# AllanYangZhou/midGPT

Hardware: AMD Instinct MI355X
Metric: tokens_per_sec (higher is better)
Workload: dtype bf16; 1 GPU; model=openwebtext_xl-gpt-1311M, global_batch=128, seq_len=1024, parallelism=dp1, g_accum_iters=2, remat=False

## Files before the change

midgpt_amd/ops/csrc/attention.hip:

```cpp
#include "common.h"
#include "mfma.h"
#include "philox.h"

struct AttnStrides {
  long b, h;
  int r;
};
DEVINL long bh_base(const AttnStrides& s, long bh, int H) {
  return (bh / H) * s.b + (bh % H) * s.h;
}

template <int C> DEVINL int swz_rm(int row, int byte_in_row) {
  constexpr int M = (C == 128) ? 15 : 7;
  return byte_in_row ^ ((row & M) << 4);
}
DEVINL int swz_tr(int row, int byte_in_row) {
  return byte_in_row ^ (((row >> 2) & 3) << 4);
}

template <int C, int NT>
struct RmStage {
  static constexpr int NV = (32 * C + NT * 8 - 1) / (NT * 8);
  u16x8 v[NV];
  DEVINL void load(const u16* __restrict__ g, int ld = C) {
    static_assert((NT * 8) % C == 0, "a thread keeps its column across loads");
    const int idx0 = threadIdx.x * 8;
    const unsigned boff = 2u * (unsigned)((idx0 / C) * ld + idx0 % C);
#pragma unroll
    for (int i = 0; i < NV; ++i) {
      if (idx0 + i * NT * 8 < 32 * C)
        v[i] = *(const u16x8*)((const char*)(g + (long)(i * (NT * 8 / C)) * ld) + boff);
    }
  }
  DEVINL void write(u16* lds) const {
#pragma unroll
    for (int i = 0; i < NV; ++i) {
      const int idx = threadIdx.x * 8 + i * NT * 8;
      if (idx < 32 * C) {
        const int row = idx / C, col = idx % C;
        *(u16x8*)((char*)lds + row * C * 2 + swz_rm<C>(row, col * 2)) = v[i];
      }
    }
  }
};
template <int C, int NT, bool ACCK = false>
struct TrStage {
  static constexpr int NP = (32 * C + NT * 16 - 1) / (NT * 16);
  u16x8 a[NP], b[NP];
  DEVINL void load(const u16* __restrict__ g, int ld = C) {
    static_assert((NT * 8) % C == 0, "a thread keeps its column across loads");
    const int idx0 = threadIdx.x * 16;
    const unsigned boff =
        2u * (unsigned)(2 * (idx0 / (2 * C)) * ld + (idx0 / 2) % C);
#pragma unroll
    for (int i = 0; i < NP; ++i) {
      if (idx0 + i * NT * 16 >= 32 * C) continue;
      const u16* gi = g + (long)(i * 2 * (NT * 8 / C)) * ld;
      const char* pa = (const char*)gi + boff;
      int ldb = 2 * ld;
      asm volatile("" : "+s"(ldb));
      if constexpr (ACCK) {
        unsigned off = boff;
        asm volatile("" : "+v"(off));
        a[i] = *(const u16x8*)((const char*)gi + off);
        b[i] = *(const u16x8*)((const char*)gi + ldb + off);
        continue;
      }
      a[i] = *(const u16x8*)pa;
      b[i] = *(const u16x8*)(pa + ldb);
    }
  }
  DEVINL void write_tr(u16* lds) const {
#pragma unroll
    for (int i = 0; i < NP; ++i) {
      const int idx = threadIdx.x * 16 + i * NT * 16;
      if (idx >= 32 * C) continue;
      const int row0 = 2 * (idx / (2 * C));
      const int row = ACCK ? acc_k_pos(row0) : row0;
      const int col = (idx / 2) % C;
      if constexpr (ACCK) {
        const u32x4 aw = __builtin_bit_cast(u32x4, a[i]);
        const u32x4 bw = __builtin_bit_cast(u32x4, b[i]);
        const int x = (row * 2) ^ (((col >> 3) & 1) << 5);
        char* const p0 = (char*)lds + col * 64 + x;
        char* const p1 = (char*)lds + col * 64 + (x ^ 16);
#pragma unroll
        for (int j = 0; j < 8; ++j) {
          const unsigned pv = (j & 1)
              ? (aw[j >> 1] >> 16) | (bw[j >> 1] & 0xffff0000u)
              : (aw[j >> 1] & 0xffffu) | (bw[j >> 1] << 16);
          *(unsigned*)((j < 4 ? p0 : p1) + j * 64) = pv;
        }
        continue;
      }
#pragma unroll
      for (int j = 0; j < 8; ++j) {
        const int r = col + j;
        u16x2 pv; pv.x = a[i][j]; pv.y = b[i][j];
        *(u16x2*)((char*)lds + r * 64 + swz_tr(r, row * 2)) = pv;
      }
    }
  }
  DEVINL void write_rm(u16* lds) const {
#pragma unroll
    for (int i = 0; i < NP; ++i) {
      const int idx = threadIdx.x * 16 + i * NT * 16;
      if (idx >= 32 * C) continue;
      const int row = 2 * (idx / (2 * C));
      const int col = (idx / 2) % C;
      *(u16x8*)((char*)lds + row * C * 2 + swz_rm<C>(row, col * 2)) = a[i];
      *(u16x8*)((char*)lds + (row + 1) * C * 2 + swz_rm<C>(row + 1, col * 2)) = b[i];
    }
  }
};
template <int C, int NT>
DEVINL void stage_rm(const u16* __restrict__ g, u16* lds, int ld = C) {
  RmStage<C, NT> st; st.load(g, ld); st.write(lds);
}
template <int C, int NT, bool ACCK = false>
DEVINL void stage_tr(const u16* __restrict__ g, u16* lds, int ld = C) {
  TrStage<C, NT, ACCK> st; st.load(g, ld); st.write_tr(lds);
}

template <int C>
DEVINL bf16x8_t read_rm_frag(const u16* lds, int row, int cbyte) {
  return *(const bf16x8_t*)((const char*)lds + row * C * 2 + swz_rm<C>(row, cbyte));
}
DEVINL bf16x8_t read_tr_frag(const u16* lds, int row, int kbyte) {
  return *(const bf16x8_t*)((const char*)lds + row * 64 + swz_tr(row, kbyte));
}

DEVINL float shfl32(float v, int src) { return __shfl(v, src, 32); }

template <int C, int NW, int SPW, bool DROP = false>
__global__ __launch_bounds__(NW * 64, 2) void attn_fwd_kernel(const u16* __restrict__ q,
                                const u16* __restrict__ k,
                                const u16* __restrict__ v,
                                u16* __restrict__ o, float* __restrict__ lse,
                                int B, int H, int T,
                                AttnStrides sv, AttnStrides so,
                                uint32_t seed_lo = 0, uint32_t seed_hi = 0,
                                uint32_t drop_thr = 0, float inv_keep = 1.f) {
  constexpr int NCB = C / 32;
  constexpr int NCH = C / 16;
  constexpr int NSTRIP = NW * SPW;
  const float scale = rsqrtf((float)C);
  const long bh = blockIdx.x % ((long)B * H);
  const int qb = blockIdx.x / (B * H);
  const int q0 = qb * (NSTRIP * 32);
  const int lane = lane_id();
  const int w = wave_id();
  int strip[SPW];
  strip[0] = w;
  if (SPW == 2) strip[1] = NSTRIP - 1 - w;

  extern __shared__ __attribute__((aligned(16))) char smem[];
  u16* ldsK = (u16*)smem;
  u16* ldsVt = (u16*)(smem + 2 * 32 * C * 2);
  float* obuf = (float*)smem;

  const u16* qg = q + (bh * T) * C;
  const u16* kg = k + (bh * T) * C;
  const u16* vg = v + bh_base(sv, bh, H);

  bf16x8_t qf[NCH];
  f32x16 oacc[SPW][NCB];
  float m[SPW], lsum[SPW];
  {
    const u16* qrow = qg + (long)(q0 + 32 * strip[SPW - 1] + (lane & 31)) * C;
#pragma unroll
    for (int ch = 0; ch < NCH; ++ch)
      qf[ch] = *(const bf16x8_t*)(qrow + 16 * ch + 8 * (lane >> 5));
  }
#pragma unroll
  for (int sp = 0; sp < SPW; ++sp) {
#pragma unroll
    for (int cb = 0; cb < NCB; ++cb) oacc[sp][cb] = (f32x16)(0.f);
    m[sp] = -1e30f;
    lsum[sp] = 0.f;
  }

  const int nkt = (q0 + NSTRIP * 32) / 32;
  stage_rm<C, NW * 64>(kg, ldsK);
  stage_tr<C, NW * 64>(vg, ldsVt, sv.r);
  __syncthreads();

  RmStage<C, NW * 64> kst;
  TrStage<C, NW * 64> vst;
  for (int kt = 0; kt < nkt; ++kt) {
    const int buf = kt & 1;
    const bool pre = kt + 1 < nkt;
    if (pre) {
      kst.load(kg + (long)(kt + 1) * 32 * C);
      vst.load(vg + (long)(kt + 1) * 32 * sv.r, sv.r);
    }
    const int k0 = kt * 32;
#pragma unroll
    for (int sp = 0; sp < SPW; ++sp) {
      const int qw0 = q0 + 32 * strip[sp];
      const int myq = qw0 + (lane & 31);
      if (k0 > qw0 + 31) continue;
      f32x16 s = (f32x16)(0.f);
      const u16* kb = ldsK + buf * 32 * C;
      const u16* qrow = qg + (long)myq * C;
#pragma unroll
      for (int ch = 0; ch < NCH; ++ch) {
        bf16x8_t a = read_rm_frag<C>(kb, lane & 31, 16 * ch * 2 + 16 * (lane >> 5));
        bf16x8_t qfr = (sp == SPW - 1) ? qf[ch]
            : *(const bf16x8_t*)(qrow + 16 * ch + 8 * (lane >> 5));
        s = mfma_32x32x16_bf16(a, qfr, s);
      }
      float sv[16];
      float mt = -1e30f;
#pragma unroll
      for (int r = 0; r < 16; ++r) {
        sv[r] = (k0 + mfma_d_row(lane, r) > myq) ? -1e30f : s[r];
        mt = fmaxf(mt, sv[r]);
      }
      mt = fmaxf(mt, __shfl_xor(mt, 32));
      const float mn = fmaxf(m[sp], mt);
      const float alpha = __expf((m[sp] - mn) * scale);
      const bool need_rescale = !__all(mt <= m[sp]);
      m[sp] = mn;
      float p[16], psum = 0.f;
#pragma unroll
      for (int r = 0; r < 16; ++r) {
        p[r] = __expf((sv[r] - mn) * scale);
        psum += p[r];
      }
      psum += __shfl_xor(psum, 32);
      lsum[sp] = lsum[sp] * alpha + psum;
      if (need_rescale) {
        float arow[16];
#pragma unroll
        for (int r = 0; r < 16; ++r) arow[r] = shfl32(alpha, mfma_d_row(lane, r));
#pragma unroll
        for (int cb = 0; cb < NCB; ++cb)
#pragma unroll
// ... 32 lines not shown
      vst.write_tr(ldsVt + (1 - buf) * C * 32);
    }
    __syncthreads();
  }

#pragma unroll
  for (int sp = 0; sp < SPW; ++sp) {
    const int qw0 = q0 + 32 * strip[sp];
    const int myq = qw0 + (lane & 31);
    float rec = 1.f / lsum[sp];
    if constexpr (DROP) rec *= inv_keep;
    float rrow[16];
#pragma unroll
    for (int r = 0; r < 16; ++r) rrow[r] = shfl32(rec, mfma_d_row(lane, r));
    if (lane < 32) lse[bh * T + myq] = m[sp] * scale + __logf(lsum[sp]);
    float* ob = obuf + w * 32 * 32;
    u16* og = o + bh_base(so, bh, H) + (long)qw0 * so.r;
#pragma unroll
    for (int cb = 0; cb < NCB; ++cb) {
#pragma unroll
      for (int r = 0; r < 16; ++r) {
        const int row = mfma_d_row(lane, r);
        *(float*)((char*)ob + row * 128 + (((lane & 31) * 4) ^ ((row & 7) << 4))) =
            oacc[sp][cb][r] * rrow[r];
      }
      __builtin_amdgcn_s_waitcnt(0);
      const int row = lane & 31;
      const int c16 = 16 * (lane >> 5);
      float tmp[16];
#pragma unroll
      for (int i = 0; i < 4; ++i) {
        f32x4 t = *(const f32x4*)((char*)ob + row * 128 + (((c16 + 4 * i) * 4) ^ ((row & 7) << 4)));
        tmp[4 * i] = t[0]; tmp[4 * i + 1] = t[1]; tmp[4 * i + 2] = t[2]; tmp[4 * i + 3] = t[3];
      }
      u16x8 out0, out1;
#pragma unroll
      for (int j = 0; j < 8; ++j) { out0[j] = f2b(tmp[j]); out1[j] = f2b(tmp[8 + j]); }
      *(u16x8*)(og + (long)row * so.r + 32 * cb + c16) = out0;
      *(u16x8*)(og + (long)row * so.r + 32 * cb + c16 + 8) = out1;
      __builtin_amdgcn_s_waitcnt(0);
    }
  }
}

template <int C, int NW>
__global__ __launch_bounds__(NW * 64, 2) void attn_fwd2_kernel(
    const u16* __restrict__ q, const u16* __restrict__ k,
    const u16* __restrict__ v, u16* __restrict__ o, float* __restrict__ lse,
    int B, int H, int T, AttnStrides sv, AttnStrides so) {
  constexpr int NCB = C / 32;
  constexpr int NCH = C / 16;
  const float scale = rsqrtf((float)C);
  const long bh = blockIdx.x % ((long)B * H);
  const int qb = blockIdx.x / (B * H);
  const int q0 = qb * (NW * 32);
  const int lane = lane_id();
  const int w = wave_id();
  const int qw0 = q0 + 32 * w;
  const int myq = qw0 + (lane & 31);

  extern __shared__ __attribute__((aligned(16))) char smem[];
  u16* ldsK = (u16*)smem;
  u16* ldsVt = (u16*)(smem + 2 * 64 * C * 2);
  float* obuf = (float*)smem;

  const u16* qg = q + (bh * T) * C;
  const u16* kg = k + (bh * T) * C;
  const u16* vg = v + bh_base(sv, bh, H);

  bf16x8_t qf[NCH];
  {
    const u16* qrow = qg + (long)myq * C;
#pragma unroll
    for (int ch = 0; ch < NCH; ++ch)
      qf[ch] = *(const bf16x8_t*)(qrow + 16 * ch + 8 * (lane >> 5));
  }
  f32x16 oacc[NCB];
#pragma unroll
  for (int cb = 0; cb < NCB; ++cb) oacc[cb] = (f32x16)(0.f);
  float m = -1e30f, lsum = 0.f;

  const int nrounds = (q0 + NW * 32) / 64;
  stage_rm<C, NW * 64>(kg, ldsK);
  stage_rm<C, NW * 64>(kg + 32 * C, ldsK + 32 * C);
  stage_tr<C, NW * 64>(vg, ldsVt, sv.r);
  stage_tr<C, NW * 64>(vg + (long)32 * sv.r, ldsVt + C * 32, sv.r);
  __syncthreads();

  RmStage<C, NW * 64> kstA, kstB;
  TrStage<C, NW * 64> vstA, vstB;
  for (int rd = 0; rd < nrounds; ++rd) {
    const int buf = rd & 1;
    const bool pre = rd + 1 < nrounds;
    if (pre) {
      const long nb = (long)(rd + 1) * 64;
      kstA.load(kg + nb * C);
      kstB.load(kg + (nb + 32) * C);
      vstA.load(vg + nb * sv.r, sv.r);
      vstB.load(vg + (nb + 32) * sv.r, sv.r);
    }
    const int k0 = rd * 64;
    if (k0 <= qw0 + 31) {
      const u16* kbuf = ldsK + buf * 64 * C;
      const u16* vbuf = ldsVt + buf * 64 * C;
      const bool needB = (k0 + 32) <= qw0 + 31;
      f32x16 s0 = (f32x16)(0.f), s1 = (f32x16)(0.f);
#pragma unroll
      for (int ch = 0; ch < NCH; ++ch) {
        bf16x8_t a0 = read_rm_frag<C>(kbuf, lane & 31, 16 * ch * 2 + 16 * (lane >> 5));
        s0 = mfma_32x32x16_bf16(a0, qf[ch], s0);
      }
      if (needB) {
#pragma unroll
        for (int ch = 0; ch < NCH; ++ch) {
          bf16x8_t a1 = read_rm_frag<C>(kbuf + 32 * C, lane & 31,
                                        16 * ch * 2 + 16 * (lane >> 5));
          s1 = mfma_32x32x16_bf16(a1, qf[ch], s1);
        }
      }
      float sv0[16], sv1[16];
      float mt = -1e30f;
#pragma unroll
      for (int r = 0; r < 16; ++r) {
        sv0[r] = (k0 + mfma_d_row(lane, r) > myq) ? -1e30f : s0[r];
        mt = fmaxf(mt, sv0[r]);
        sv1[r] = (!needB || k0 + 32 + mfma_d_row(lane, r) > myq) ? -1e30f : s1[r];
        mt = fmaxf(mt, sv1[r]);
      }
      mt = fmaxf(mt, __shfl_xor(mt, 32));
      const float mn = fmaxf(m, mt);
      const float alpha = __expf((m - mn) * scale);
      const bool need_rescale = !__all(mt <= m);
      m = mn;
      float p0[16], p1[16], psum = 0.f;
#pragma unroll
      for (int r = 0; r < 16; ++r) {
        p0[r] = __expf((sv0[r] - mn) * scale);
        p1[r] = __expf((sv1[r] - mn) * scale);
        psum += p0[r] + p1[r];
      }
// ... 99 lines not shown
      bh = urow / (unsigned)T;
      t = urow % (unsigned)T;
    }
    const u16* dor = dO + bh_base(sdo, bh, H) + t * sdo.r;
    const u16* orow = O + bh_base(so, bh, H) + t * so.r;
    float acc = 0.f;
    const u16x8 a = *(const u16x8*)(dor + i);
    const u16x8 b = *(const u16x8*)(orow + i);
    if (do_copy) *(u16x8*)(do_copy + (bh * T + t) * C + i) = a;
#pragma unroll
    for (int j = 0; j < 8; ++j) acc += b2f(a[j]) * b2f(b[j]);
    acc = group_sum<LPR>(acc);
    if (lane % LPR == 0) delta[bh * T + t] = acc;
  }
}

template <int C, int NW>
constexpr bool attn_dkv_vf_lds = !(C == 128 && NW == 4);
template <int C, int NW>
constexpr int attn_dkv_kf_lds = C == 128 ? 3 : 0;

template <int C, int NW, bool DROP = false>
__global__ __launch_bounds__(NW * 64, 2) void attn_bwd_dkv_kernel(
    const u16* __restrict__ dO, const u16* __restrict__ q,
    const u16* __restrict__ k, const u16* __restrict__ v,
    const float* __restrict__ lse, const float* __restrict__ delta,
    u16* __restrict__ dk, u16* __restrict__ dv, int B, int H, int T,
    AttnStrides sdo, AttnStrides sv, AttnStrides sdv,
    uint32_t seed_lo = 0, uint32_t seed_hi = 0, uint32_t drop_thr = 0,
    float inv_keep = 1.f) {
  constexpr int NCB = C / 32;
  constexpr int NCH = C / 16;
  constexpr int TILE = 4 * 32 * C;
  const float scale = rsqrtf((float)C);
  const long bh = blockIdx.x % ((long)B * H);
  const int kb = blockIdx.x / (B * H);
  const int lane = lane_id();
  const int w = wave_id();
  const int kw0 = kb * (NW * 32) + 32 * w;
  const int myk = kw0 + (lane & 31);

  extern __shared__ __attribute__((aligned(16))) char smem[];
  u16* base = (u16*)smem;
  float* ldsLse = (float*)(base + 2 * TILE);
  float* ldsDelta = ldsLse + 64;
  constexpr bool VF_LDS = attn_dkv_vf_lds<C, NW>;
  bf16x8_t* ldsVf = (bf16x8_t*)(ldsDelta + 64) + w * (NCH * 64) + lane;

  const u16* qg = q + (bh * T) * C;
  const u16* kg = k + (bh * T) * C;
  const u16* vg = v + bh_base(sv, bh, H);
  const u16* dog = dO + bh_base(sdo, bh, H);
  const u16* krow = kg + (long)myk * C;
  const u16* vrow = vg + (long)myk * sv.r;
  if constexpr (VF_LDS) {
#pragma unroll
    for (int ch = 0; ch < NCH; ++ch)
      ldsVf[ch * 64] = *(const bf16x8_t*)(vrow + 16 * ch + 8 * (lane >> 5));
  }

  constexpr bool KF_RES = !(DROP && C == 128);
  constexpr int NKL = KF_RES ? attn_dkv_kf_lds<C, NW> : 0;
  constexpr int NKR = KF_RES ? NCH - NKL : 0;
  bf16x8_t kf[NKR ? NKR : 1];
  bf16x8_t* ldsKf = (bf16x8_t*)(ldsDelta + 64) + (VF_LDS ? NW * (NCH * 64) : 0) +
                    w * (NKL * 64) + lane;
  if (KF_RES) {
#pragma unroll
    for (int ch = 0; ch < NCH; ++ch) {
      const bf16x8_t f = *(const bf16x8_t*)(krow + 16 * ch + 8 * (lane >> 5));
      if (ch < NKR) kf[ch < NKR ? ch : 0] = f;
      else ldsKf[(ch - NKR) * 64] = f;
    }
  }

  f32x16 dvacc[NCB], dkacc[NCB];
#pragma unroll
  for (int cb = 0; cb < NCB; ++cb) { dvacc[cb] = (f32x16)(0.f); dkacc[cb] = (f32x16)(0.f); }

  const int qt0 = kb * NW;
  const int nqt = T / 32;

  auto stage_set = [&](int qt, int buf) {
    const long qbase = (long)qt * 32;
    u16* bq = base + buf * TILE;
    stage_rm<C, NW * 64>(qg + qbase * C, bq);
    stage_tr<C, NW * 64, true>(qg + qbase * C, bq + 32 * C);
    stage_rm<C, NW * 64>(dog + qbase * sdo.r, bq + 2 * 32 * C, sdo.r);
    stage_tr<C, NW * 64, true>(dog + qbase * sdo.r, bq + 3 * 32 * C, sdo.r);
    if (threadIdx.x < 32) {
      ldsLse[buf * 32 + threadIdx.x] = lse[bh * T + qbase + threadIdx.x];
      ldsDelta[buf * 32 + threadIdx.x] = delta[bh * T + qbase + threadIdx.x];
    }
  };

  stage_set(qt0, 0);
  __syncthreads();
  __builtin_amdgcn_s_waitcnt(0);
  TrStage<C, NW * 64, true> qst, dost;
  float lse_r = 0.f, del_r = 0.f;
  for (int qt = qt0; qt < nqt; ++qt) {
    const int buf = (qt - qt0) & 1;
    const bool pre = qt + 1 < nqt;
    if (pre) {
      const long nb = (long)(qt + 1) * 32;
      qst.load(qg + nb * C);
      dost.load(dog + nb * sdo.r, sdo.r);
      if (threadIdx.x < 32) {
        unsigned off = 4u * threadIdx.x;
        asm volatile("" : "+v"(off));
        lse_r = *(const float*)((const char*)(lse + bh * T + nb) + off);
        del_r = *(const float*)((const char*)(delta + bh * T + nb) + off);
      }
    }
    const int qbase = qt * 32;
    if (qbase + 31 >= kw0) {
      const u16* ldsQ = base + buf * TILE;
      const u16* ldsQt = ldsQ + 32 * C;
      const u16* ldsDO = ldsQt + C * 32;
      const u16* ldsDOt = ldsDO + 32 * C;
      const float* lseb = ldsLse + buf * 32;
      const float* deltab = ldsDelta + buf * 32;
      uint32_t keep = 0;
      if constexpr (DROP) {
#pragma unroll
        for (int g = 0; g < 4; ++g)
          keep |= attn_drop_keep4(seed_lo, seed_hi, (uint32_t)bh,
                                  (uint32_t)(qbase + 8 * g + 4 * (lane >> 5)) >> 2,
                                  (uint32_t)myk, drop_thr) << (4 * g);
        __builtin_amdgcn_sched_barrier(0);
      }
      f32x16 s = (f32x16)(0.f);
#pragma unroll
      for (int ch = 0; ch < NCH; ++ch) {
        bf16x8_t a = read_rm_frag<C>(ldsQ, lane & 31, 16 * ch * 2 + 16 * (lane >> 5));
        bf16x8_t kfr;
        if constexpr (!KF_RES) kfr = *(const bf16x8_t*)(krow + 16 * ch + 8 * (lane >> 5));
        else if (ch < NKR) kfr = kf[ch < NKR ? ch : 0];
        else kfr = ldsKf[(ch - NKR) * 64];
        s = mfma_32x32x16_bf16(a, kfr, s);
      }
      float p[16];
#pragma unroll
      for (int g = 0; g < 4; ++g) {
        const f32x4 l4 = *(const f32x4*)(lseb + 8 * g + 4 * (lane >> 5));
#pragma unroll
        for (int i = 0; i < 4; ++i) {
          const int r = 4 * g + i;
          const int qrow = qbase + mfma_d_row(lane, r);
          p[r] = (myk > qrow) ? 0.f : __expf(s[r] * scale - l4[i]);
        }
      }
      const bf16x8_t pf0 = dlayout_pack(p, DROP ? keep : 0xffu);
      const bf16x8_t pf1 = dlayout_pack(p + 8, DROP ? keep >> 8 : 0xffu);
#pragma unroll
      for (int cb = 0; cb < NCB; ++cb) {
        bf16x8_t b0 = read_tr_frag(ldsDOt, 32 * cb + (lane & 31), 16 * (lane >> 5));
        bf16x8_t b1 = read_tr_frag(ldsDOt, 32 * cb + (lane & 31), 32 + 16 * (lane >> 5));
        dvacc[cb] = mfma_32x32x16_bf16(pf0, b0, dvacc[cb]);
        dvacc[cb] = mfma_32x32x16_bf16(pf1, b1, dvacc[cb]);
      }
      f32x16 dp = (f32x16)(0.f);
#pragma unroll
      for (int ch = 0; ch < NCH; ++ch) {
        bf16x8_t a = read_rm_frag<C>(ldsDO, lane & 31, 16 * ch * 2 + 16 * (lane >> 5));
        bf16x8_t vf;
        if constexpr (VF_LDS) vf = ldsVf[ch * 64];
        else vf = *(const bf16x8_t*)(vrow + 16 * ch + 8 * (lane >> 5));
        dp = mfma_32x32x16_bf16(a, vf, dp);
      }
      float ds[16];
#pragma unroll
      for (int g = 0; g < 4; ++g) {
        const f32x4 d4 = *(const f32x4*)(deltab + 8 * g + 4 * (lane >> 5));
#pragma unroll
        for (int i = 0; i < 4; ++i) {
          const int r = 4 * g + i;
          float dpr = dp[r];
          if constexpr (DROP) dpr = ((keep >> r) & 1u) ? dpr * inv_keep : 0.f;
          ds[r] = p[r] * (dpr - d4[i]) * scale;
        }
      }
      const bf16x8_t df0 = dlayout_pack(ds);
      const bf16x8_t df1 = dlayout_pack(ds + 8);
#pragma unroll
      for (int cb = 0; cb < NCB; ++cb) {
        bf16x8_t b0 = read_tr_frag(ldsQt, 32 * cb + (lane & 31), 16 * (lane >> 5));
        bf16x8_t b1 = read_tr_frag(ldsQt, 32 * cb + (lane & 31), 32 + 16 * (lane >> 5));
        dkacc[cb] = mfma_32x32x16_bf16(df0, b0, dkacc[cb]);
        dkacc[cb] = mfma_32x32x16_bf16(df1, b1, dkacc[cb]);
      }
    }
    if (pre) {
      u16* bq = base + (buf ^ 1) * TILE;
      qst.write_rm(bq);
      qst.write_tr(bq + 32 * C);
      dost.write_rm(bq + 2 * 32 * C);
      dost.write_tr(bq + 3 * 32 * C);
      if (threadIdx.x < 32) {
        ldsLse[(buf ^ 1) * 32 + threadIdx.x] = lse_r;
        ldsDelta[(buf ^ 1) * 32 + threadIdx.x] = del_r;
      }
    }
    __syncthreads();
  }

  float* ob = (float*)smem + w * 32 * 32;
  u16* dkg = dk + (bh * T + kw0) * C;
  u16* dvg = dv + bh_base(sdv, bh, H) + (long)kw0 * sdv.r;
#pragma unroll
  for (int which = 0; which < 2; ++which) {
    f32x16* acc = which == 0 ? dkacc : dvacc;
    u16* out = which == 0 ? dkg : dvg;
    const int old = which == 0 ? C : sdv.r;
#pragma unroll
    for (int cb = 0; cb < NCB; ++cb) {
#pragma unroll
      for (int r = 0; r < 16; ++r) {
        const int row = mfma_d_row(lane, r);
        float a = acc[cb][r];
        if constexpr (DROP) { if (which == 1) a *= inv_keep; }
        *(float*)((char*)ob + row * 128 + (((lane & 31) * 4) ^ ((row & 7) << 4))) = a;
      }
      __builtin_amdgcn_s_waitcnt(0);
      const int row = lane & 31;
      const int c16 = 16 * (lane >> 5);
      float tmp[16];
#pragma unroll
      for (int i = 0; i < 4; ++i) {
        f32x4 t = *(const f32x4*)((char*)ob + row * 128 +
                                  (((c16 + 4 * i) * 4) ^ ((row & 7) << 4)));
        tmp[4 * i] = t[0]; tmp[4 * i + 1] = t[1];
        tmp[4 * i + 2] = t[2]; tmp[4 * i + 3] = t[3];
      }
      u16x8 o0, o1;
#pragma unroll
      for (int j = 0; j < 8; ++j) { o0[j] = f2b(tmp[j]); o1[j] = f2b(tmp[8 + j]); }
// ... 181 lines not shown
```

midgpt_amd/ops/csrc/bindings.cpp:

```cpp
#include <torch/extension.h>
#include <hip/hip_runtime.h>
#include <c10/hip/HIPGuard.h>
#include <c10/hip/HIPStream.h>

#include <algorithm>
#include <climits>
#include <type_traits>
#include <vector>

static hipStream_t cur_stream() { return c10::hip::getCurrentHIPStream().stream(); }

template <typename... P, typename... A>
static void launch(void (*kernel)(P...), dim3 grid, int block, size_t smem, A... args) {
  if (grid.x == 0 || grid.y == 0 || grid.z == 0) return;
  if (smem > 64 * 1024) {
    hipError_t e = hipFuncSetAttribute(reinterpret_cast<const void*>(kernel),
                                       hipFuncAttributeMaxDynamicSharedMemorySize, (int)smem);
    TORCH_CHECK(e == hipSuccess, "cannot raise dynamic LDS to ", smem, " bytes: ",
                hipGetErrorString(e));
  }
  hipLaunchKernelGGL(kernel, grid, dim3(block), smem, cur_stream(), static_cast<P>(args)...);
  hipError_t e = hipGetLastError();
  TORCH_CHECK(e == hipSuccess, "HIP launch failed: ", hipGetErrorString(e));
}
// ... 23 lines not shown
      if (sizes[i] != ANY && sizes[i] != ts[i]) return false;
    return true;
  }
};
static Shape flat(int64_t n) {
  Shape s((at::IntArrayRef()));
  s.numel = n;
  return s;
}
static std::ostream& operator<<(std::ostream& o, const Shape& s) {
  return s.numel >= 0 ? o << s.numel << " elements" : o << "shape " << s.sizes << " (-1: any)";
}

template <typename T>
static T* fresh(const torch::Tensor& t) {
  return static_cast<T*>(t.data_ptr());
}

struct Call {
  const char* who;
  int dev;
  c10::hip::OptionalHIPGuard guard;

  static int device_of(const char* who, const torch::Tensor& first) {
    TORCH_CHECK(first.defined() && first.is_cuda(), who, ": the first tensor must be on the GPU");
    return first.get_device();
  }
  Call(const char* who, const torch::Tensor& first) : who(who), dev(device_of(who, first)) {
    if (dev != c10::hip::current_device()) guard.set_index((c10::DeviceIndex)dev);
  }

  template <typename T, c10::ScalarType ST>
  T* ptr(const torch::Tensor& t, const char* name, const Shape& s) const {
    TORCH_CHECK(t.defined() && t.is_cuda() && t.get_device() == dev,
                who, ": ", name, " must be a tensor on GPU ", dev);
    TORCH_CHECK(t.is_contiguous() && t.scalar_type() == ST && s.fits(t),
                who, ": ", name, " must be contiguous ", ST, " of ", s, ", got ",
                t.scalar_type(), " ", t.sizes(), t.is_contiguous() ? "" : " (strided)");
    return static_cast<T*>(t.data_ptr());
  }
  const u16* bf16(const torch::Tensor& t, const char* n, const Shape& s) const {
    return ptr<u16, torch::kBFloat16>(t, n, s);
  }
  u16* bf16_out(const torch::Tensor& t, const char* n, const Shape& s) const {
    return ptr<u16, torch::kBFloat16>(t, n, s);
  }
  const float* f32(const torch::Tensor& t, const char* n, const Shape& s) const {
    return ptr<float, torch::kFloat>(t, n, s);
  }
  float* f32_out(const torch::Tensor& t, const char* n, const Shape& s) const {
    return ptr<float, torch::kFloat>(t, n, s);
  }
  const long* i64(const torch::Tensor& t, const char* n, const Shape& s) const {
    return ptr<long, torch::kLong>(t, n, s);
  }
  const int* i32(const torch::Tensor& t, const char* n, const Shape& s) const {
    return ptr<int, torch::kInt>(t, n, s);
  }
  const u16* bf16(const c10::optional<torch::Tensor>& t, const char* n, const Shape& s) const {
    return t.has_value() ? bf16(*t, n, s) : nullptr;
  }
  int dim(const torch::Tensor& t, int i) const {
    const int64_t n = t.sizes()[i];
    TORCH_CHECK(n <= INT_MAX, who, ": a dimension of ", n, " does not fit int");
    return (int)n;
  }
};

std::vector<torch::Tensor> rmsnorm_fwd(torch::Tensor x, c10::optional<torch::Tensor> w,
                                       double eps) {
  Call c("rmsnorm_fwd", x);
  const bool fp32 = x.scalar_type() == torch::kFloat;
  const float* xf = fp32 ? c.f32(x, "x", {ANY, ANY}) : nullptr;
  const u16* xb = fp32 ? nullptr : c.bf16(x, "x", {ANY, ANY});
  long N = x.size(0);
  int D = c.dim(x, 1);
  TORCH_CHECK(fp32 || D % 8 == 0, "rmsnorm_fwd: bf16 rows need D % 8 == 0");
  auto y = torch::empty_like(x);
  auto invrms = torch::empty({N}, x.options().dtype(torch::kFloat));
  const float* wp = nullptr;
  torch::Tensor wf;
  if (w.has_value()) {
    wf = w->to(torch::kFloat).contiguous();
    wp = c.f32(wf, "w", flat(D));
  }
  int rows_per_block = 4;
  long grid = std::min((N + rows_per_block - 1) / rows_per_block, (long)8192);
  if (fp32)
    launch(rmsnorm_fwd_kernel<float, 1>, grid, 256, 0, xf, wp, fresh<float>(y),
           fresh<float>(invrms), N, D, (float)eps);
  else
    launch(rmsnorm_fwd_bf16, grid, 256, 0, xb, wp, fresh<u16>(y), fresh<float>(invrms), N, D,
           (float)eps);
  return {y, invrms};
}

std::vector<torch::Tensor> rmsnorm_bwd(torch::Tensor dy, torch::Tensor x,
                                       c10::optional<torch::Tensor> w,
                                       torch::Tensor invrms, double eps) {
  Call c("rmsnorm_bwd", dy);
  TORCH_CHECK(!w.has_value(), "rmsnorm_bwd: weighted path unimplemented on HIP "
                              "(the model's norms are weightless)");
  const u16* xp = c.bf16(x, "x", {ANY, ANY});
  long N = x.size(0);
  int D = c.dim(x, 1);
  TORCH_CHECK(D % 8 == 0, "rmsnorm_bwd: D % 8 == 0 required");
// ... 891 lines not shown
  auto out = torch::empty({(long)B}, logits.options().dtype(torch::kLong));
  const bool has_k = top_k >= 1 && top_k < V;
  const uint64_t s = (uint64_t)seed;
  dispatch_flag(has_k, [&](auto hk) {
    launch(sample_tokens_kernel<decltype(hk)::value>, B, SAMPLE_THREADS, 0, lp,
           fresh<long>(out), V, it, has_k ? (int)top_k : 0, (uint32_t)s, (uint32_t)(s >> 32),
           (uint32_t)step);
  });
  return out;
}

torch::Tensor sample_tokens_rows(torch::Tensor logits, torch::Tensor params_dev,
                                 torch::Tensor inv_t, torch::Tensor top_k, torch::Tensor seeds,
                                 torch::Tensor steps, torch::Tensor rows) {
  Call c("sample_tokens_rows", logits);
  const u16* lp = c.bf16(logits, "logits", {ANY, ANY});
  const int B = c.dim(logits, 0), V = c.dim(logits, 1);
  TORCH_CHECK(V >= 1, "sample_tokens_rows: empty rows");
  TORCH_CHECK(!inv_t.is_cuda() && inv_t.dim() == 1 && inv_t.size(0) == B &&
              inv_t.scalar_type() == torch::kFloat,
              c.who, ": inv_t must be a CPU float32 tensor of ", B, " values");
  auto itc = inv_t.contiguous();
  for (int b = 0; b < B; ++b) {
    const float it = itc.data_ptr<float>()[b];
    TORCH_CHECK(std::isfinite(it) && it >= 0.f, c.who,
                ": inv_t must be finite and > 0, or 0 for a greedy row, got ", it);
  }
  for (int64_t k : host_lens(top_k, B, c.who))
    TORCH_CHECK(k >= 0, c.who, ": top_k >= 0 required (0: all), got ", k);
  host_lens(seeds, B, c.who);
  for (int64_t s : host_lens(steps, B, c.who))
    TORCH_CHECK(s >= 0 && s <= (int64_t)UINT32_MAX, c.who, ": step must be in [0, 2^32), got ", s);
  for (int64_t r : host_lens(rows, B, c.who))
    TORCH_CHECK(r >= 0 && r <= (int64_t)UINT32_MAX, c.who, ": row must be in [0, 2^32), got ", r);
  const int* pp = c.i32(params_dev, "params_dev", {B, SAMPLE_ROW_WORDS});
  auto out = torch::empty({(long)B}, logits.options().dtype(torch::kLong));
  launch(sample_tokens_rows_kernel, B, SAMPLE_THREADS, 0, lp, fresh<long>(out), V, pp);
  return out;
}

torch::Tensor probe_mfma(torch::Tensor A, torch::Tensor B) {
  Call c("probe_mfma", A);
  const float *ap = c.f32(A, "A", {32, 16}), *bp = c.f32(B, "B", {16, 32});
  auto D = torch::zeros({32, 32}, A.options());
  launch(probe_mfma_kernel, 1, 64, 0, ap, bp, fresh<float>(D));
  return D;
}
torch::Tensor probe_pack(torch::Tensor M, torch::Tensor B) {
  Call c("probe_pack", M);
  const float *mp = c.f32(M, "M", {32, 32}), *bp = c.f32(B, "B", {32, 32});
  auto D = torch::zeros({32, 32}, M.options());
  launch(probe_pack_kernel, 1, 64, 0, mp, bp, fresh<float>(D));
  return D;
}

#include "blaslt.inc"

PYBIND11_MODULE(TORCH_EXTENSION_NAME, mod) {
  mod.def("rmsnorm_fwd", &rmsnorm_fwd);
  mod.def("rmsnorm_bwd", &rmsnorm_bwd);
  mod.def("qkv_prep_fwd", &qkv_prep_fwd);
  mod.def("qkv_prep_bwd", &qkv_prep_bwd);
  mod.def("add_rmsnorm_fwd", &add_rmsnorm_fwd);
  mod.def("add_rmsnorm_bwd", &add_rmsnorm_bwd);
  mod.def("qk_prep_fwd", &qk_prep_fwd);
  mod.def("qk_prep_bwd", &qk_prep_bwd);
  mod.def("ce_fwd", &ce_fwd);
  mod.def("ce_bwd", &ce_bwd);
  mod.def("adamw_step", &adamw_step);
  mod.def("attn_fwd", &attn_fwd);
  mod.def("attn_bwd", &attn_bwd);
  mod.def("attn_delta", &attn_delta, py::arg("dO"), py::arg("o"), py::arg("bthc"));
  mod.def("attn_fwd_dropout", &attn_fwd_dropout);
  mod.def("attn_bwd_dropout", &attn_bwd_dropout);
  mod.def("attn_fwd_packed", &attn_fwd_packed, py::arg("q"), py::arg("k"),
          py::arg("v"), py::arg("p") = 0.0, py::arg("seed") = 0);
  mod.def("attn_bwd_packed", &attn_bwd_packed, py::arg("dO"), py::arg("q"),
          py::arg("k"), py::arg("v"), py::arg("o"), py::arg("lse"),
          py::arg("dqkv"), py::arg("p") = 0.0, py::arg("seed") = 0,
          py::arg("stage_do") = true);
  mod.def("kv_append", &kv_append, py::arg("qkv"), py::arg("qw"), py::arg("kw"),
          py::arg("sin"), py::arg("cos"), py::arg("k_cache"), py::arg("v_cache"),
          py::arg("pos"), py::arg("eps") = 1e-6);
  mod.def("attn_decode", &attn_decode, py::arg("q"), py::arg("k_cache"),
          py::arg("v_cache"), py::arg("kv_len"), py::arg("num_splits") = 0);
  mod.def("kv_append_ragged", &kv_append_ragged, py::arg("qkv"), py::arg("qw"),
          py::arg("kw"), py::arg("sin"), py::arg("cos"), py::arg("k_cache"),
          py::arg("v_cache"), py::arg("pos_dev"), py::arg("pos_host"),
          py::arg("eps") = 1e-6);
  mod.def("attn_decode_ragged", &attn_decode_ragged, py::arg("q"), py::arg("k_cache"),
          py::arg("v_cache"), py::arg("kv_lens_dev"), py::arg("kv_lens_host"),
          py::arg("num_splits") = 0);
  mod.def("kv_append_slots", &kv_append_slots, py::arg("qkv"), py::arg("qw"), py::arg("kw"),
          py::arg("sin"), py::arg("cos"), py::arg("k_cache"), py::arg("v_cache"),
          py::arg("pos_dev"), py::arg("pos_host"), py::arg("slots_dev"),
          py::arg("slots_host"), py::arg("eps") = 1e-6);
  mod.def("attn_decode_slots", &attn_decode_slots, py::arg("q"), py::arg("k_cache"),
          py::arg("v_cache"), py::arg("kv_lens_dev"), py::arg("kv_lens_host"),
          py::arg("slots_dev"), py::arg("slots_host"), py::arg("num_splits") = 0);
  mod.def("kv_append_paged", &kv_append_paged, py::arg("qkv"), py::arg("qw"), py::arg("kw"),
          py::arg("sin"), py::arg("cos"), py::arg("k_pool"), py::arg("v_pool"),
          py::arg("pos_dev"), py::arg("pos_host"), py::arg("block_table_dev"),
          py::arg("block_table_host"), py::arg("eps") = 1e-6);
  mod.def("attn_decode_paged", &attn_decode_paged, py::arg("q"), py::arg("k_pool"),
          py::arg("v_pool"), py::arg("kv_lens_dev"), py::arg("kv_lens_host"),
          py::arg("block_table_dev"), py::arg("block_table_host"), py::arg("num_splits") = 0);
  mod.def("kv_store_paged", &kv_store_paged, py::arg("k"), py::arg("v"), py::arg("k_pool"),
          py::arg("v_pool"), py::arg("lens_dev"), py::arg("lens_host"),
          py::arg("block_table_dev"), py::arg("block_table_host"));
  mod.def("attn_decode_auto_splits", &attn_decode_auto_splits, py::arg("rows"),
          py::arg("kv_len"), py::arg("cus"));
  mod.def("sample_tokens", &sample_tokens, py::arg("logits"), py::arg("inv_t"),
          py::arg("top_k"), py::arg("seed"), py::arg("step"));
  mod.def("sample_tokens_rows", &sample_tokens_rows, py::arg("logits"), py::arg("params_dev"),
          py::arg("inv_t"), py::arg("top_k"), py::arg("seeds"), py::arg("steps"),
          py::arg("rows"));
  mod.def("embedding_bwd", &embedding_bwd);
  mod.def("gelu_fwd", &gelu_fwd);
  mod.def("gelu_bwd", &gelu_bwd);
  mod.def("transpose_batched", &transpose_batched, py::arg("src"), py::arg("dst"),
          py::arg("table_dev"), py::arg("table_host"), py::arg("max_blocks") = 0);
  mod.def("lt_probe", &lt_probe);
  mod.def("matmul_dgelu", &matmul_dgelu);
  mod.def("probe_mfma", &probe_mfma);
  mod.def("probe_pack", &probe_pack);
}
```

midgpt_amd/ops/csrc/mfma.h:

```cpp
#pragma once
#include "common.h"

using bf16x8_t = __attribute__((ext_vector_type(8))) __bf16;

DEVINL f32x16 mfma_32x32x16_bf16(bf16x8_t a, bf16x8_t b, f32x16 c) {
  return __builtin_amdgcn_mfma_f32_32x32x16_bf16(a, b, c, 0, 0, 0);
}

DEVINL int mfma_d_row(int lane, int r) {
  return (r & 3) + 8 * (r >> 2) + 4 * (lane >> 5);
}

DEVINL unsigned pack_bf16(float lo, float hi) {
  return ((unsigned)f2b(hi) << 16) | (unsigned)f2b(lo);
}

DEVINL int acc_k_pos(int i) {
  return (i & ~12) | ((i & 4) << 1) | ((i & 8) >> 1);
}

DEVINL bf16x8_t dlayout_pack(const float* s , unsigned keep8 = 0xffu) {
  union { unsigned u[4]; bf16x8_t v; } out;
#pragma unroll
  for (int i = 0; i < 4; ++i) {
    const unsigned mk = (((keep8 >> (2 * i)) & 1u) ? 0x0000ffffu : 0u) |
                        (((keep8 >> (2 * i + 1)) & 1u) ? 0xffff0000u : 0u);
    out.u[i] = pack_bf16(s[2 * i], s[2 * i + 1]) & mk;
  }
  return out.v;
}

DEVINL bf16x8_t dlayout_to_afrag(const float* s ) {
  unsigned x0 = pack_bf16(s[0], s[1]);
  unsigned x1 = pack_bf16(s[2], s[3]);
  unsigned x2 = pack_bf16(s[4], s[5]);
  unsigned x3 = pack_bf16(s[6], s[7]);
  {
    auto r = __builtin_amdgcn_permlane32_swap(x0, x2, false, false);
    x0 = r[0]; x2 = r[1];
  }
  {
    auto r = __builtin_amdgcn_permlane32_swap(x1, x3, false, false);
    x1 = r[0]; x3 = r[1];
  }
  union { unsigned u[4]; bf16x8_t v; } out;
  out.u[0] = x0; out.u[1] = x1; out.u[2] = x2; out.u[3] = x3;
  return out.v;
}
```

midgpt_amd/ops/csrc/probe.hip:

```cpp
#include "common.h"
#include "mfma.h"

__global__ void probe_mfma_kernel(const float* __restrict__ A,
                                  const float* __restrict__ B,
                                  float* __restrict__ D) {
  const int lane = threadIdx.x;
  bf16x8_t a, b;
#pragma unroll
  for (int j = 0; j < 8; ++j) {
    a[j] = (__bf16)A[(lane & 31) * 16 + 8 * (lane >> 5) + j];
    b[j] = (__bf16)B[(8 * (lane >> 5) + j) * 32 + (lane & 31)];
  }
  f32x16 d = (f32x16)(0.f);
  d = mfma_32x32x16_bf16(a, b, d);
#pragma unroll
  for (int r = 0; r < 16; ++r)
    D[mfma_d_row(lane, r) * 32 + (lane & 31)] = d[r];
}

__global__ void probe_pack_kernel(const float* __restrict__ M,
                                  const float* __restrict__ B,
                                  float* __restrict__ D) {
  const int lane = threadIdx.x;
  float m[16];
#pragma unroll
  for (int r = 0; r < 16; ++r)
    m[r] = M[mfma_d_row(lane, r) * 32 + (lane & 31)];
  bf16x8_t a0 = dlayout_to_afrag(m);
  bf16x8_t a1 = dlayout_to_afrag(m + 8);
  bf16x8_t b0, b1;
#pragma unroll
  for (int j = 0; j < 8; ++j) {
    b0[j] = (__bf16)B[(8 * (lane >> 5) + j) * 32 + (lane & 31)];
    b1[j] = (__bf16)B[(16 + 8 * (lane >> 5) + j) * 32 + (lane & 31)];
  }
  f32x16 d = (f32x16)(0.f);
  d = mfma_32x32x16_bf16(a0, b0, d);
  d = mfma_32x32x16_bf16(a1, b1, d);
#pragma unroll
  for (int r = 0; r < 16; ++r)
    D[mfma_d_row(lane, r) * 32 + (lane & 31)] = d[r];
}
```

Measured before the change: 121,000 tokens/s.

## Tune attention kernels: reverse causal block order, packed bf16 convert, scheduling barriers

Several unrelated attention tweaks land together. The staging loops are split into unconditional full iterations plus one guarded tail, and the transpose write always uses the word-packed path. The second forward kernel launches the heaviest causal query blocks first, and pack_bf16 uses a vector convert that may lower to a packed bf16 conversion instruction. The backward pass adds sched_barriers and asm pins around the P and dS packs and keeps V loads as offsets. Extra waitcnts after the initial barriers and a bf16 pack probe kernel are also added. The changed non-ACCK transpose write path may not match the old swz_tr layout.

Result: faster. 124,800 tokens/s, median of 6 (+3.2%).

```diff
diff --git a/midgpt_amd/ops/csrc/attention.hip b/midgpt_amd/ops/csrc/attention.hip
--- a/midgpt_amd/ops/csrc/attention.hip
+++ b/midgpt_amd/ops/csrc/attention.hip
@@ -21,95 +21,103 @@
 template <int C, int NT>
 struct RmStage {
   static constexpr int NV = (32 * C + NT * 8 - 1) / (NT * 8);
+  static constexpr int NF = (32 * C) / (NT * 8);
   u16x8 v[NV];
+  DEVINL void load1(const u16* __restrict__ g, int ld, unsigned boff, int i) {
+    v[i] = *(const u16x8*)((const char*)(g + (long)(i * (NT * 8 / C)) * ld) + boff);
+  }
   DEVINL void load(const u16* __restrict__ g, int ld = C) {
     static_assert((NT * 8) % C == 0, "a thread keeps its column across loads");
     const int idx0 = threadIdx.x * 8;
     const unsigned boff = 2u * (unsigned)((idx0 / C) * ld + idx0 % C);
 #pragma unroll
-    for (int i = 0; i < NV; ++i) {
-      if (idx0 + i * NT * 8 < 32 * C)
-        v[i] = *(const u16x8*)((const char*)(g + (long)(i * (NT * 8 / C)) * ld) + boff);
-    }
+    for (int i = 0; i < NF; ++i) load1(g, ld, boff, i);
+    if constexpr (NV > NF) {
+      if (idx0 + NF * NT * 8 < 32 * C) load1(g, ld, boff, NF);
+    }
+  }
+  DEVINL void write1(u16* lds, int i) const {
+    const int idx = threadIdx.x * 8 + i * NT * 8;
+    const int row = idx / C, col = idx % C;
+    *(u16x8*)((char*)lds + row * C * 2 + swz_rm<C>(row, col * 2)) = v[i];
   }
   DEVINL void write(u16* lds) const {
 #pragma unroll
-    for (int i = 0; i < NV; ++i) {
-      const int idx = threadIdx.x * 8 + i * NT * 8;
-      if (idx < 32 * C) {
-        const int row = idx / C, col = idx % C;
-        *(u16x8*)((char*)lds + row * C * 2 + swz_rm<C>(row, col * 2)) = v[i];
-      }
+    for (int i = 0; i < NF; ++i) write1(lds, i);
+    if constexpr (NV > NF) {
+      if ((int)threadIdx.x * 8 + NF * NT * 8 < 32 * C) write1(lds, NF);
     }
   }
 };
 template <int C, int NT, bool ACCK = false>
 struct TrStage {
   static constexpr int NP = (32 * C + NT * 16 - 1) / (NT * 16);
+  static constexpr int NF = (32 * C) / (NT * 16);
+  static DEVINL bool mine(int i) { return (int)threadIdx.x * 16 + i * NT * 16 < 32 * C; }
   u16x8 a[NP], b[NP];
+  DEVINL void load1(const u16* __restrict__ g, int ld, unsigned boff, int i) {
+    const u16* gi = g + (long)(i * 2 * (NT * 8 / C)) * ld;
+    int ldb = 2 * ld;
+    asm volatile("" : "+s"(ldb));
+    if constexpr (ACCK) {
+      unsigned off = boff;
+      asm volatile("" : "+v"(off));
+      a[i] = *(const u16x8*)((const char*)gi + off);
+      b[i] = *(const u16x8*)((const char*)gi + ldb + off);
+    } else {
+      const char* pa = (const char*)gi + boff;
+      a[i] = *(const u16x8*)pa;
+      b[i] = *(const u16x8*)(pa + ldb);
+    }
+  }
   DEVINL void load(const u16* __restrict__ g, int ld = C) {
     static_assert((NT * 8) % C == 0, "a thread keeps its column across loads");
     const int idx0 = threadIdx.x * 16;
     const unsigned boff =
         2u * (unsigned)(2 * (idx0 / (2 * C)) * ld + (idx0 / 2) % C);
 #pragma unroll
-    for (int i = 0; i < NP; ++i) {
-      if (idx0 + i * NT * 16 >= 32 * C) continue;
-      const u16* gi = g + (long)(i * 2 * (NT * 8 / C)) * ld;
-      const char* pa = (const char*)gi + boff;
-      int ldb = 2 * ld;
-      asm volatile("" : "+s"(ldb));
-      if constexpr (ACCK) {
-        unsigned off = boff;
-        asm volatile("" : "+v"(off));
-        a[i] = *(const u16x8*)((const char*)gi + off);
-        b[i] = *(const u16x8*)((const char*)gi + ldb + off);
-        continue;
-      }
-      a[i] = *(const u16x8*)pa;
-      b[i] = *(const u16x8*)(pa + ldb);
+    for (int i = 0; i < NF; ++i) load1(g, ld, boff, i);
+    if constexpr (NP > NF) {
+      if (mine(NF)) load1(g, ld, boff, NF);
+    }
+  }
+  DEVINL void write_tr1(u16* lds, int i) const {
+    const int idx = threadIdx.x * 16 + i * NT * 16;
+    const int row0 = 2 * (idx / (2 * C));
+    const int row = ACCK ? acc_k_pos(row0) : row0;
+    const int col = (idx / 2) % C;
+    const u32x4 aw = __builtin_bit_cast(u32x4, a[i]);
+    const u32x4 bw = __builtin_bit_cast(u32x4, b[i]);
+    const int x = (row * 2) ^ (((col >> 3) & 1) << 5);
+    char* const p0 = (char*)lds + col * 64 + x;
+    char* const p1 = (char*)lds + col * 64 + (x ^ 16);
+#pragma unroll
+    for (int j = 0; j < 8; ++j) {
+      const unsigned pv = (j & 1)
+          ? (aw[j >> 1] >> 16) | (bw[j >> 1] & 0xffff0000u)
+          : (aw[j >> 1] & 0xffffu) | (bw[j >> 1] << 16);
+      *(unsigned*)((j < 4 ? p0 : p1) + j * 64) = pv;
     }
   }
   DEVINL void write_tr(u16* lds) const {
 #pragma unroll
-    for (int i = 0; i < NP; ++i) {
-      const int idx = threadIdx.x * 16 + i * NT * 16;
-      if (idx >= 32 * C) continue;
-      const int row0 = 2 * (idx / (2 * C));
-      const int row = ACCK ? acc_k_pos(row0) : row0;
-      const int col = (idx / 2) % C;
-      if constexpr (ACCK) {
-        const u32x4 aw = __builtin_bit_cast(u32x4, a[i]);
-        const u32x4 bw = __builtin_bit_cast(u32x4, b[i]);
-        const int x = (row * 2) ^ (((col >> 3) & 1) << 5);
-        char* const p0 = (char*)lds + col * 64 + x;
-        char* const p1 = (char*)lds + col * 64 + (x ^ 16);
-#pragma unroll
-        for (int j = 0; j < 8; ++j) {
-          const unsigned pv = (j & 1)
-              ? (aw[j >> 1] >> 16) | (bw[j >> 1] & 0xffff0000u)
-              : (aw[j >> 1] & 0xffffu) | (bw[j >> 1] << 16);
-          *(unsigned*)((j < 4 ? p0 : p1) + j * 64) = pv;
-        }
-        continue;
-      }
-#pragma unroll
-      for (int j = 0; j < 8; ++j) {
-        const int r = col + j;
-        u16x2 pv; pv.x = a[i][j]; pv.y = b[i][j];
-        *(u16x2*)((char*)lds + r * 64 + swz_tr(r, row * 2)) = pv;
-      }
-    }
+    for (int i = 0; i < NF; ++i) write_tr1(lds, i);
+    if constexpr (NP > NF) {
+      if (mine(NF)) write_tr1(lds, NF);
+    }
+  }
+  DEVINL void write_rm1(u16* lds, int i) const {
+    const int idx = threadIdx.x * 16 + i * NT * 16;
+    const int row = 2 * (idx / (2 * C));
+    const int col = (idx / 2) % C;
+    *(u16x8*)((char*)lds + row * C * 2 + swz_rm<C>(row, col * 2)) = a[i];
+    *(u16x8*)((char*)lds + (row + 1) * C * 2 + swz_rm<C>(row + 1, col * 2)) = b[i];
   }
   DEVINL void write_rm(u16* lds) const {
 #pragma unroll
-    for (int i = 0; i < NP; ++i) {
-      const int idx = threadIdx.x * 16 + i * NT * 16;
-      if (idx >= 32 * C) continue;
-      const int row = 2 * (idx / (2 * C));
-      const int col = (idx / 2) % C;
-      *(u16x8*)((char*)lds + row * C * 2 + swz_rm<C>(row, col * 2)) = a[i];
-      *(u16x8*)((char*)lds + (row + 1) * C * 2 + swz_rm<C>(row + 1, col * 2)) = b[i];
+    for (int i = 0; i < NF; ++i) write_rm1(lds, i);
+    if constexpr (NP > NF) {
+      if (mine(NF)) write_rm1(lds, NF);
     }
   }
 };
@@ -184,6 +192,7 @@
   stage_rm<C, NW * 64>(kg, ldsK);
   stage_tr<C, NW * 64>(vg, ldsVt, sv.r);
   __syncthreads();
+  __builtin_amdgcn_s_waitcnt(0);
 
   RmStage<C, NW * 64> kst;
   TrStage<C, NW * 64> vst;
@@ -322,7 +331,7 @@
   constexpr int NCH = C / 16;
   const float scale = rsqrtf((float)C);
   const long bh = blockIdx.x % ((long)B * H);
-  const int qb = blockIdx.x / (B * H);
+  const int qb = T / (NW * 32) - 1 - blockIdx.x / (B * H);
   const int q0 = qb * (NW * 32);
   const int lane = lane_id();
   const int w = wave_id();
@@ -356,6 +365,7 @@
   stage_tr<C, NW * 64>(vg, ldsVt, sv.r);
   stage_tr<C, NW * 64>(vg + (long)32 * sv.r, ldsVt + C * 32, sv.r);
   __syncthreads();
+  __builtin_amdgcn_s_waitcnt(0);
 
   RmStage<C, NW * 64> kstA, kstB;
   TrStage<C, NW * 64> vstA, vstB;
@@ -561,8 +571,9 @@
   const u16* vg = v + bh_base(sv, bh, H);
   const u16* dog = dO + bh_base(sdo, bh, H);
   const u16* krow = kg + (long)myk * C;
-  const u16* vrow = vg + (long)myk * sv.r;
+  const unsigned vrow_off = 2u * (unsigned)(myk * sv.r + 8 * (lane >> 5));
   if constexpr (VF_LDS) {
+    const u16* vrow = vg + (long)myk * sv.r;
 #pragma unroll
     for (int ch = 0; ch < NCH; ++ch)
       ldsVf[ch * 64] = *(const bf16x8_t*)(vrow + 16 * ch + 8 * (lane >> 5));
@@ -660,8 +671,10 @@
           p[r] = (myk > qrow) ? 0.f : __expf(s[r] * scale - l4[i]);
         }
       }
-      const bf16x8_t pf0 = dlayout_pack(p, DROP ? keep : 0xffu);
-      const bf16x8_t pf1 = dlayout_pack(p + 8, DROP ? keep >> 8 : 0xffu);
+      bf16x8_t pf0 = dlayout_pack(p, DROP ? keep : 0xffu);
+      bf16x8_t pf1 = dlayout_pack(p + 8, DROP ? keep >> 8 : 0xffu);
+      asm volatile("" : "+v"(pf0), "+v"(pf1));
+      __builtin_amdgcn_sched_barrier(0);
 #pragma unroll
       for (int cb = 0; cb < NCB; ++cb) {
         bf16x8_t b0 = read_tr_frag(ldsDOt, 32 * cb + (lane & 31), 16 * (lane >> 5));
@@ -674,8 +687,13 @@
       for (int ch = 0; ch < NCH; ++ch) {
         bf16x8_t a = read_rm_frag<C>(ldsDO, lane & 31, 16 * ch * 2 + 16 * (lane >> 5));
         bf16x8_t vf;
-        if constexpr (VF_LDS) vf = ldsVf[ch * 64];
-        else vf = *(const bf16x8_t*)(vrow + 16 * ch + 8 * (lane >> 5));
+        if constexpr (VF_LDS) {
+          vf = ldsVf[ch * 64];
+        } else {
+          unsigned off = vrow_off;
+          asm volatile("" : "+v"(off));
+          vf = *(const bf16x8_t*)((const char*)vg + off + 32 * ch);
+        }
         dp = mfma_32x32x16_bf16(a, vf, dp);
       }
       float ds[16];
@@ -690,8 +708,10 @@
           ds[r] = p[r] * (dpr - d4[i]) * scale;
         }
       }
-      const bf16x8_t df0 = dlayout_pack(ds);
-      const bf16x8_t df1 = dlayout_pack(ds + 8);
+      bf16x8_t df0 = dlayout_pack(ds);
+      bf16x8_t df1 = dlayout_pack(ds + 8);
+      asm volatile("" : "+v"(df0), "+v"(df1));
+      __builtin_amdgcn_sched_barrier(0);
 #pragma unroll
       for (int cb = 0; cb < NCB; ++cb) {
         bf16x8_t b0 = read_tr_frag(ldsQt, 32 * cb + (lane & 31), 16 * (lane >> 5));
diff --git a/midgpt_amd/ops/csrc/bindings.cpp b/midgpt_amd/ops/csrc/bindings.cpp
--- a/midgpt_amd/ops/csrc/bindings.cpp
+++ b/midgpt_amd/ops/csrc/bindings.cpp
@@ -99,6 +99,9 @@
     return ptr<float, torch::kFloat>(t, n, s);
   }
   const long* i64(const torch::Tensor& t, const char* n, const Shape& s) const {
+    return ptr<long, torch::kLong>(t, n, s);
+  }
+  long* i64_out(const torch::Tensor& t, const char* n, const Shape& s) const {
     return ptr<long, torch::kLong>(t, n, s);
   }
   const int* i32(const torch::Tensor& t, const char* n, const Shape& s) const {
@@ -1096,6 +1099,16 @@
   auto D = torch::zeros({32, 32}, M.options());
   launch(probe_pack_kernel, 1, 64, 0, mp, bp, fresh<float>(D));
   return D;
+}
+void probe_bf16_pack(torch::Tensor counts, int64_t start, int64_t n) {
+  Call c("probe_bf16_pack", counts);
+  long* cp = c.i64_out(counts, "counts", {3});
+  TORCH_CHECK(start >= 0 && start <= (int64_t)UINT32_MAX && n >= 0 && n <= (1LL << 32),
+              "probe_bf16_pack: start in [0, 2^32) and n in [0, 2^32] required, got ", start,
+              " and ", n);
+  const long grid = std::min((long)((n + 255) / 256), 4096L);
+  launch(probe_bf16_pack_kernel, grid, 256, 0, (uint32_t)start, (unsigned long long)n,
+         reinterpret_cast<unsigned long long*>(cp));
 }
 
 #include "blaslt.inc"
@@ -1168,4 +1181,5 @@
   mod.def("matmul_dgelu", &matmul_dgelu);
   mod.def("probe_mfma", &probe_mfma);
   mod.def("probe_pack", &probe_pack);
-}
+  mod.def("probe_bf16_pack", &probe_bf16_pack);
+}
diff --git a/midgpt_amd/ops/csrc/mfma.h b/midgpt_amd/ops/csrc/mfma.h
--- a/midgpt_amd/ops/csrc/mfma.h
+++ b/midgpt_amd/ops/csrc/mfma.h
@@ -11,8 +11,10 @@
   return (r & 3) + 8 * (r >> 2) + 4 * (lane >> 5);
 }
 
+using bf16x2_t = __attribute__((ext_vector_type(2))) __bf16;
 DEVINL unsigned pack_bf16(float lo, float hi) {
-  return ((unsigned)f2b(hi) << 16) | (unsigned)f2b(lo);
+  const f32x2 v = {lo, hi};
+  return __builtin_bit_cast(unsigned, __builtin_convertvector(v, bf16x2_t));
 }
 
 DEVINL int acc_k_pos(int i) {
diff --git a/midgpt_amd/ops/csrc/probe.hip b/midgpt_amd/ops/csrc/probe.hip
--- a/midgpt_amd/ops/csrc/probe.hip
+++ b/midgpt_amd/ops/csrc/probe.hip
@@ -41,3 +41,28 @@
   for (int r = 0; r < 16; ++r)
     D[mfma_d_row(lane, r) * 32 + (lane & 31)] = d[r];
 }
+
+__global__ void probe_bf16_pack_kernel(uint32_t start, unsigned long long n,
+                                       unsigned long long* __restrict__ counts) {
+  auto bits = [](uint32_t u) { return __builtin_bit_cast(float, u); };
+  auto is_nan16 = [](uint32_t h) { return (h & 0x7fffu) > 0x7f80u; };
+  unsigned long long bad = 0, bad_nan = 0, lost_nan = 0;
+  const unsigned long long step = (unsigned long long)gridDim.x * blockDim.x;
+  for (unsigned long long i = (unsigned long long)blockIdx.x * blockDim.x + threadIdx.x;
+       i < n; i += step) {
+    const uint32_t x = start + (uint32_t)i;
+    const unsigned lo = pack_bf16(bits(x), bits(~x));
+    const unsigned hi = pack_bf16(bits(~x), bits(x));
+    const uint32_t want = f2b(bits(x));
+    const bool same = (lo & 0xffffu) == want && (hi >> 16) == want;
+    if ((x & 0x7fffffffu) > 0x7f800000u) {
+      bad_nan += !same;
+      lost_nan += !(is_nan16(lo & 0xffffu) && is_nan16(hi >> 16));
+    } else {
+      bad += !same;
+    }
+  }
+  if (bad) atomicAdd(&counts[0], bad);
+  if (bad_nan) atomicAdd(&counts[1], bad_nan);
+  if (lost_nan) atomicAdd(&counts[2], lost_nan);
+}
```
